# ruc-aimc-lab/GeoFormer

Measured on AMD Instinct MI355X. Metric: image-pairs/sec (640x640), higher is better.
Workload: dtype f16

## Files before the change

geoformer_amd/csrc/k10_conv3x3.hip:

```cpp
#include <type_traits>

#include "gf_common.h"

namespace {

constexpr int TW = 32, PW = TW + 2;
constexpr int C10_FRAG = 1024;
constexpr int P_OFF = 0;
enum { C10_NONE = 0, C10_RELU = 1, C10_LEAKY = 2 };

struct ConvArgs {
    const void* x;
    const void* wstream;
    const float* shift;
    const void* res;
    void* out;
    const void* zeros;
    int N, H, W, act;
    float slope;
    int tiles_x, tiles_y, ntiles;
    int Hi, Wi;
};

template <int NT, int NW, bool REM = false, bool S2 = false>
struct ConvGeo {
    static constexpr int PB = NT <= 4 ? 2 : 1;
    static constexpr int TH = NW * PB, PH = S2 ? TH + 1 : TH + 2;
    static constexpr int PIECES = (PH * PW + 15) / 16;
    static constexpr int PLANE_BYTES = PIECES * 1024;
    static constexpr int PATCH_BYTES = S2 ? 4 * PLANE_BYTES : PIECES * 1024;
    static constexpr int W10_OFF = S2 ? PATCH_BYTES : 2 * PATCH_BYTES;
    static_assert(!S2 || PB == 1, "the stride-2 form is built for the wide outputs (one row per wave)");
#ifndef K10_BS
#define K10_BS 6
#endif
    static constexpr int BLOCK_STEPS = S2 ? 3 : (NW == 8 && PB == 1) ? K10_BS : 6;
    static constexpr int FR = BLOCK_STEPS * NT;
    static constexpr int WBLK = FR * C10_FRAG;
    static constexpr int SHIFT_OFF = W10_OFF + 2 * WBLK;
    static constexpr int RPIECES = (PH * PW + 63) / 64;
    static constexpr int R_OFF = SHIFT_OFF + NT * 32 * 4 + 16;
    static constexpr int LDS = R_OFF + (REM ? RPIECES * 1024 : 0);
    static_assert(LDS <= 160 * 1024, "LDS budget");
};

struct ConvRsrc {
    __amdgpu_buffer_rsrc_t r;
};
__device__ __forceinline__ ConvRsrc conv_rsrc(const void* p, unsigned bytes) {
    return ConvRsrc{__builtin_amdgcn_make_buffer_rsrc(const_cast<void*>(p), 0, (int)bytes, 0x00020000)};
}
__device__ __forceinline__ void conv_lds_dma(const ConvRsrc& rs, char* dst, int voffset, int soffset) {
    __builtin_amdgcn_raw_ptr_buffer_load_lds(rs.r, (__attribute__((address_space(3))) void*)dst, 16, voffset, soffset, 0, 0);
}
template <int NT, int NW, bool S2 = false>
__device__ __forceinline__ void conv_dma_block(const ConvRsrc& ws, char* smem, int b, int slot, int wave, int lane, int i0 = 0, int i1 = 1 << 20) {
    using G = ConvGeo<NT, NW, false, S2>;
    asm volatile("" : "+v"(lane));
    char* dst = smem + G::W10_OFF + slot * G::WBLK;
#pragma unroll
    for (int i = 0; i < (G::FR + NW - 1) / NW; ++i) {
        const int f = wave + NW * i;
        if (i >= i0 && i < i1 && (NW * (i + 1) <= G::FR || f < G::FR)) conv_lds_dma(ws, dst + f * C10_FRAG, lane * 16, b * G::WBLK + f * C10_FRAG);
    }
}

template <typename T, int CIN, int NT, int NW>
__device__ __forceinline__ void conv_dma_patch(const ConvArgs& a, const ConvRsrc& xs, char* smem, int buf, int n, int y0, int x0, int c, int wave,
                                               int lane, int i0 = 0, int i1 = 1 << 20) {
    using G = ConvGeo<NT, NW>;
    asm volatile("" : "+v"(lane));
    char* dst = smem + P_OFF + buf * G::PATCH_BYTES;
    const int sbase = ((n * a.Hi + y0 - 1) * a.Wi + x0 - 1) * CIN + 32 * c;
#pragma unroll
    for (int i = 0; i < (G::PIECES + NW - 1) / NW; ++i) {
        const int piece = wave + NW * i;
        if (i >= i0 && i < i1 && (NW * (i + 1) <= G::PIECES || piece < G::PIECES)) {
            const int q = piece * 16 + (lane >> 2), slot = (lane & 3) ^ ((q >> 1) & 3);
            const int pr = q / PW, pc = q - pr * PW;
            const bool in = (unsigned)(y0 - 1 + pr) < (unsigned)a.Hi && (unsigned)(x0 - 1 + pc) < (unsigned)a.Wi && q < G::PH * PW;
            int off = (sbase + (pr * a.Wi + pc) * CIN + 8 * slot) * (int)sizeof(T);
            asm volatile("" : "+v"(off));
            conv_lds_dma(xs, dst + piece * 1024, in ? off : 0x7FFFFFF0, 0);
        }
    }
}

template <typename T, int CIN, int NT, int NW>
__device__ __forceinline__ void conv_dma_plane(const ConvArgs& a, const ConvRsrc& xs, char* smem, int plane, int n, int y0, int x0, int c, int wave,
                                               int lane) {
    using G = ConvGeo<NT, NW, false, true>;
    asm volatile("" : "+v"(lane));
    char* dst = smem + P_OFF + plane * G::PLANE_BYTES;
    const int py = plane >> 1, px = plane & 1;
    const int iy0 = 2 * y0 - 1 + py, ix0 = 2 * x0 - 1 + px;
    const int sbase = ((n * a.Hi + iy0) * a.Wi + ix0) * CIN + 32 * c;
#pragma unroll
    for (int i = 0; i < (G::PIECES + NW - 1) / NW; ++i) {
        const int piece = wave + NW * i;
        if (piece < G::PIECES) {
            const int q = piece * 16 + (lane >> 2), slot = (lane & 3) ^ ((q >> 1) & 3);
            const int pr = q / PW, pc = q - pr * PW;
            const bool in = (unsigned)(iy0 + 2 * pr) < (unsigned)a.Hi && (unsigned)(ix0 + 2 * pc) < (unsigned)a.Wi && q < G::PH * PW;
            int off = (sbase + 2 * (pr * a.Wi + pc) * CIN + 8 * slot) * (int)sizeof(T);
            asm volatile("" : "+v"(off));
            conv_lds_dma(xs, dst + piece * 1024, in ? off : 0x7FFFFFF0, 0);
        }
    }
}

template <typename T, int CIN, int NT, int NW>
__device__ __forceinline__ void conv_dma_patch_rem(const ConvArgs& a, const ConvRsrc& xs, char* smem, int n, int y0, int x0, int wave, int lane) {
    using G = ConvGeo<NT, NW, true>;
    asm volatile("" : "+v"(lane));
    char* dst = smem + G::R_OFF;
    const int sbase = ((n * a.Hi + y0 - 1) * a.Wi + x0 - 1) * CIN + 192;
#pragma unroll
    for (int i = 0; i < (G::RPIECES + NW - 1) / NW; ++i) {
        const int piece = wave + NW * i;
        if (piece < G::RPIECES) {
            const int q = piece * 64 + lane;
            const int pr = q / PW, pc = q - pr * PW;
            const bool in = (unsigned)(y0 - 1 + pr) < (unsigned)a.Hi && (unsigned)(x0 - 1 + pc) < (unsigned)a.Wi && q < G::PH * PW;
            const int off = sbase + (pr * a.Wi + pc) * CIN;
            conv_lds_dma(xs, dst + piece * 1024, in ? off * (int)sizeof(T) : 0x7FFFFFF0, 0);
        }
    }
}

#ifndef K10_TRACE
#define K10_TRACE 0
#endif
#ifdef K10_EXP_NOSTORE
#define K10_STORE_OK (a.slope == 12345.f)
#else
#define K10_STORE_OK true
#endif
#if K10_TRACE
__device__ long long k10_trace[256 * 8 * 8 * 16];
#define K10_T(slot) do { if (lane == 0 && it < 8) k10_trace[((blockIdx.x * 8 + it) * 8 + wave) * 16 + (slot)] = (long long)__builtin_amdgcn_s_memtime(); } while (0)
__device__ long long k10_trace2[256 * 8 * 32];
#define K10_T2(slot) do { if (lane == 0 && it == 4 && c == 1) k10_trace2[(blockIdx.x * 8 + wave) * 32 + (slot)] = (long long)__builtin_amdgcn_s_memtime(); } while (0)
#else
#define K10_T(slot)
#define K10_T2(slot)
#endif

template <typename T, int CIN, int COUT, int NW, bool PADL, bool REM = false, bool S2 = false>
__global__ __launch_bounds__(NW * 64) void conv3x3_kernel(ConvArgs a) {
    using Mm = Mma16<T>;
    using Frag = typename Mm::Frag;
    using G = ConvGeo<COUT / 32, NW, REM, S2>;
    static_assert(!(S2 && REM), "no remainder form at stride 2");
    using V4 = gf_vec<T, 4>;
    using V8 = gf_vec<T, 8>;
    static_assert(!REM || CIN == 224, "the remainder form is built for 224-channel inputs");
    constexpr int NT = COUT / 32, NCH = REM ? 6 : CIN / 32, BS = G::BLOCK_STEPS, BPC = 18 / BS, RBPC = 6 / BS;
    constexpr int NBLK = NCH * BPC + (REM ? RBPC : 0);
    constexpr int PB = G::PB, TH = G::TH;
    constexpr int NSTORE = PB * 2 * NT;
    constexpr int WP = (G::FR + NW - 1) / NW, PP = (G::PIECES + NW - 1) / NW, PPMIN = G::PIECES / NW;
#ifndef K10_DEAL
#define K10_DEAL 0
#endif
    constexpr bool DEAL = K10_DEAL != 0;
    constexpr int WS = !DEAL ? 1 : WP <= 3 ? WP : 4, PS0 = DEAL ? WS : 0, PS = DEAL ? BS - WS : 1;
    auto wbeg = [](int k) { return k >= WS ? WP : k * (WP / WS) + (k < WP % WS ? k : WP % WS); };
    auto pbeg = [](int k) { return k >= PS ? PP : k * (PP / PS) + (k < PP % PS ? k : PP % PS); };
    extern __shared__ __attribute__((aligned(16))) char smem[];
    const int tid = threadIdx.x, lane = tid & 63, wave = __builtin_amdgcn_readfirstlane(tid >> 6);
    const int lp = lane & 15, g4 = lane >> 4;
    const ConvRsrc ws = conv_rsrc(a.wstream, (unsigned)NBLK * G::WBLK);
    const ConvRsrc xs = conv_rsrc(a.x, (unsigned)a.N * a.Hi * a.Wi * CIN * (unsigned)sizeof(T));
    const ConvRsrc rres = conv_rsrc(a.res, (unsigned)a.N * a.H * a.W * COUT * (unsigned)sizeof(T));
    const ConvRsrc rout = conv_rsrc(a.out, (unsigned)a.N * a.H * a.W * COUT * (unsigned)sizeof(T));
    typedef unsigned v4u __attribute__((ext_vector_type(4)));
    float* shiftv = reinterpret_cast<float*>(smem + G::SHIFT_OFF);
    for (int i = tid; i < COUT; i += NW * 64) shiftv[i] = a.shift ? a.shift[i] : 0.f;
    if (tid == 0) shiftv[COUT] = a.act == C10_LEAKY ? a.slope : 1.f;
    if (NW == 8 && wave >= 4) __builtin_amdgcn_s_setprio(1);

    auto decode = [&](int t, int& n, int& y0, int& x0) {
        const int per = a.tiles_x * a.tiles_y;
        n = t / per;
        const int r = t - n * per, ty = r / a.tiles_x;
        y0 = ty * TH;
        x0 = (r - ty * a.tiles_x) * TW;
    };
    const int n_none = a.N;
    const int xq0 = PB * wave * PW + lp;
    int swz = 0;
#pragma unroll
    for (int d = 0; d < 8; ++d) swz |= (g4 ^ (((xq0 + d) >> 1) & 3)) << (2 * d);
    const int xbase = xq0 * 64;
    Frag wa[NT], wb[NT], xa[2 * PB], xb[2 * PB];
    auto load_w = [&](Frag (&f)[NT], int slot, int s, bool second_half) {
        const char* p = smem + G::W10_OFF + slot * G::WBLK + s * NT * C10_FRAG + lane * 16;
#pragma unroll
        for (int t = 0; t < NT; ++t)
            if (!(PADL && second_half && t == NT - 1)) f[t] = *reinterpret_cast<const Frag*>(p + t * C10_FRAG);
    };
    auto load_x = [&](Frag (&f)[2 * PB], int buf, int tap) {
        constexpr int s2_plane[9] = {0, 0, 0, 0, 1, 1, 2, 2, 3}, s2_dy[9] = {0, 0, 1, 1, 0, 1, 0, 0, 0}, s2_dx[9] = {0, 1, 0, 1, 0, 0, 0, 1, 0};
        const int ky = S2 ? s2_dy[tap] : tap / 3, kx = S2 ? s2_dx[tap] : tap - 3 * (tap / 3);
        const char* p = smem + P_OFF + (S2 ? s2_plane[tap] * G::PLANE_BYTES : buf * G::PATCH_BYTES);
#ifndef K10_SWZ_TABLE
#define K10_SWZ_TABLE 1
#endif
        if constexpr (K10_SWZ_TABLE != 0) {
            int tb = swz, xb = xbase;
            asm volatile("" : "+v"(tb), "+v"(xb));
#pragma unroll
            for (int bb = 0; bb < 2 * PB; ++bb) {
                const int c = ((bb >> 1) + ky) * PW + 16 * (bb & 1) + kx;
                const int slot = __builtin_amdgcn_ubfe(tb, 2 * (c & 7), 2);
                f[bb] = *reinterpret_cast<const Frag*>(p + (xb + (slot << 4)) + c * 64);
            }
        } else {
        int xq = xq0;
        asm volatile("" : "+v"(xq));
#pragma unroll
        for (int bb = 0; bb < 2 * PB; ++bb) {
            const int q = xq + ((bb >> 1) + ky) * PW + 16 * (bb & 1) + kx;
            f[bb] = *reinterpret_cast<const Frag*>(p + q * 64 + ((g4 ^ ((q >> 1) & 3)) << 4));
        }
        }
    };

    auto load_xr = [&](Frag (&f)[2 * PB], int ks) {
        const char* p = smem + G::R_OFF;
        int xq = xq0;
        asm volatile("" : "+v"(xq));
// ... 19 lines not shown
        decode(tile0, n, y0, x0);
        if constexpr (S2) {
#pragma unroll
            for (int pl = 0; pl < 4; ++pl) conv_dma_plane<T, CIN, NT, NW>(a, xs, smem, pl, n, y0, x0, 0, wave, lane);
        } else {
            conv_dma_patch<T, CIN, NT, NW>(a, xs, smem, 0, n, y0, x0, 0, wave, lane);
        }
        conv_dma_block<NT, NW, S2>(ws, smem, 0, 0, wave, lane);
        conv_dma_block<NT, NW, S2>(ws, smem, 1, 1, wave, lane);
        asm volatile("s_waitcnt vmcnt(0) lgkmcnt(0)" ::: "memory");
        __syncthreads();
    }
    int it = -1;
    for (int tile = tile0; tile < xend; tile += xper) {
        int n, y0, x0;
        decode(tile, n, y0, x0);
        const int nxt_tile = tile + xper;
        const bool has_next = nxt_tile < xend;
        int n2 = n_none, y2 = 0, x2 = 0;
        if (has_next) decode(nxt_tile, n2, y2, x2);
        ++it;
        K10_T(0);
        load_w(wa, wslot, 0, false);
        load_x(xa, pbuf, 0);
        v4f acc[2 * PB][2 * NT];
        int il = lane;
        asm volatile("" : "+v"(il));
#pragma unroll
        for (int ct = 0; ct < 2 * NT; ++ct) {
            const float4 sh = *reinterpret_cast<const float4*>(shiftv + 32 * (ct >> 1) + 4 * (ct & 1) + 8 * (il >> 4));
#pragma unroll
            for (int bb = 0; bb < 2 * PB; ++bb) acc[bb][ct] = v4f{sh.x, sh.y, sh.z, sh.w};
        }
        auto chunk = [&](auto rem_c, int c) {
            constexpr bool R = decltype(rem_c)::value;
            constexpr int NTS = R ? 6 : 18;
            const int blk0 = R ? NCH * BPC : c * BPC;
            const bool tile_ends = R || (!REM && c + 1 == NCH);
            const bool rem_next = !R && REM && c + 1 == NCH;
#pragma unroll
            for (int ts = 0; ts < NTS; ++ts) {
                const int tap = ts >> 1, hf = ts & 1;
                Frag (&cw)[NT] = (ts & 1) ? wb : wa;
                Frag (&nw)[NT] = (ts & 1) ? wa : wb;
                Frag (&cx)[2 * PB] = (tap & 1) ? xb : xa;
                Frag (&nx)[2 * PB] = (tap & 1) ? xa : xb;
                const int kslot = (ts + 1) % BS;
                if constexpr (!R) K10_T2(ts);
                auto dma_slot = [&]() {
                    if (kslot < WS && !(ts == NTS - 1 && tile_ends)) {
                        if (ts >= BS - 1 || R || c > 0) {
                            const int nb = blk0 + (ts + 1) / BS + 1;
                            conv_dma_block<NT, NW, S2>(ws, smem, nb < NBLK ? nb : has_next ? nb - NBLK : NBLK, wslot ^ 1, wave, lane, wbeg(kslot), wbeg(kslot + 1));
                        }
                    }
                    if constexpr (S2) {
                        if (kslot == 0 && ts >= 8) {
                            const bool same = c + 1 < NCH;
                            conv_dma_plane<T, CIN, NT, NW>(a, xs, smem, (ts - 8) / 3, same ? n : n2, same ? y0 : y2, same ? x0 : x2, same ? c + 1 : 0, wave, lane);
                        }
                    } else if (!R && ts >= BS - 1 + PS0 && ts < BS - 1 + PS0 + PS) {
                        const int kp = ts - (BS - 1 + PS0);
                        const bool same = c + 1 < NCH;
                        conv_dma_patch<T, CIN, NT, NW>(a, xs, smem, pbuf ^ 1, same ? n : n2, same ? y0 : y2, same ? x0 : x2, same ? c + 1 : 0,
                                                       wave, lane, pbeg(kp), pbeg(kp + 1));
                        if constexpr (REM) {
                            if (c == 0 && kp == PS - 1) conv_dma_patch_rem<T, CIN, NT, NW>(a, xs, smem, n, y0, x0, wave, lane);
                        }
                    }
                };
                if (kslot == 0) {
                    const bool first_turn = !R && ts == BS - 1 && c == 0;
                    if (first_turn) K10_T(12);
                    if (first_turn && it > 0) asm volatile("s_waitcnt vmcnt(%0)" ::"n"(NSTORE) : "memory");
                    else if (!S2 && !R && ts == 2 * BS - 1) asm volatile("s_waitcnt vmcnt(%0)" ::"n"(PPMIN) : "memory");
                    else if (S2 && (ts >= 11 || (ts == BS - 1 && c > 0))) asm volatile("s_waitcnt vmcnt(%0)" ::"n"(PPMIN) : "memory");
                    else asm volatile("s_waitcnt vmcnt(0)" ::: "memory");
                    if (first_turn) K10_T(13);
                    if constexpr (!R) K10_T2(20 + ts / BS);
                    __builtin_amdgcn_s_barrier();
#ifdef K10_STAGGER
                    if (NW == 8 && wave >= 4) __builtin_amdgcn_s_sleep(K10_STAGGER);
#endif
                    if constexpr (!R) K10_T2(24 + ts / BS);
                    if (first_turn) K10_T(14);
                    wslot ^= 1;
                    if (ts == NTS - 1 && tile_ends) {
                        const int nb = blk0 + ts / BS + 2;
                        conv_dma_block<NT, NW, S2>(ws, smem, has_next ? nb - NBLK : NBLK, wslot ^ 1, wave, lane);
                    }
                    if (!DEAL) {
                        dma_slot();
                        if (first_turn) K10_T(15);
                    }
                    __builtin_amdgcn_sched_barrier(0);
                }
                if (DEAL && wave < 4) {
                    dma_slot();
                    __builtin_amdgcn_sched_barrier(0);
                }
                if (ts < NTS - 1 || !tile_ends) {
                    load_w(nw, wslot, (ts + 1) % BS, ((ts + 1) & 1) != 0);
                    if (hf) {
                        if constexpr (R) {
                            if (ts < NTS - 1) load_xr(nx, tap + 1);
                        } else {
                            if (ts < NTS - 1) load_x(nx, pbuf, tap + 1);
                            else if (rem_next) load_xr(nx, 0);
                            else load_x(nx, pbuf ^ 1, 0);
                        }
                    }
                }
#pragma unroll
                for (int bb = 0; bb < 2 * PB; ++bb)
#pragma unroll
                    for (int t = 0; t < NT; ++t)
                        if (!(PADL && hf == 1 && t == NT - 1)) Mm::mma(cw[t], cx[bb], acc[bb][hf * NT + t]);
                if (DEAL && wave >= 4) {
                    __builtin_amdgcn_sched_barrier(0);
                    dma_slot();
                }
                __builtin_amdgcn_sched_barrier(0);
            }
            if (!tile_ends) {
#pragma unroll
                for (int bb = 0; bb < 2 * PB; ++bb) xa[bb] = xb[bb];
            }
            if constexpr (!R) pbuf ^= 1;
            if constexpr (!R) K10_T2(18);
        };
#pragma unroll 1
        for (int c = 0; c < NCH; ++c) {
            chunk(std::integral_constant<bool, false>{}, c);
            K10_T(2 + c);
        }
        if constexpr (REM) chunk(std::integral_constant<bool, true>{}, NCH);
        K10_T(10);
        auto epilogue = [&](auto has_res_c, auto mode_c) {
            constexpr bool HAS_RES = decltype(has_res_c)::value;
            constexpr int MODE = decltype(mode_c)::value;
            int el = lane;
            asm volatile("" : "+v"(el));
            const float neg_k = MODE == 3 ? shiftv[COUT + (el >> 6)] : 1.f;
            const int odd = el & 1, ey = y0 + PB * wave;
            const int exa = x0 + (el & 14), exo = x0 + (el & 15);
            const int ebase = ((n * a.H + ey) * a.W + x0) * COUT * (int)sizeof(T) + 16 * (el >> 4);
#ifndef K10_XCHG_WIDE
#define K10_XCHG_WIDE 1
#endif
            constexpr int NB = 2 * PB, NM = (PB == 2 || K10_XCHG_WIDE) ? NT / 2 : 0, NL = NT - 2 * NM;
            constexpr bool LONE = NL != 0;
            int voa[NB], vob[NB], vol[LONE ? NB : 1];
#pragma unroll
            for (int bb = 0; bb < NB; ++bb) {
                const int rowoff = ((bb >> 1) * a.W + 16 * (bb & 1)) * COUT * (int)sizeof(T);
                const bool iny = ey + (bb >> 1) < a.H;
                voa[bb] = iny && exa + 16 * (bb & 1) < a.W ? ebase + rowoff + (el & 14) * COUT * (int)sizeof(T) + 64 * odd : 0x7FFFFFF0;
                vob[bb] = iny && exa + 1 + 16 * (bb & 1) < a.W ? ebase + rowoff + ((el & 14) + 1) * COUT * (int)sizeof(T) + 64 * odd : 0x7FFFFFF0;
                if constexpr (LONE) vol[bb] = iny && exo + 16 * (bb & 1) < a.W ? ebase + rowoff + (el & 15) * COUT * (int)sizeof(T) + 64 * (2 * NM) : 0x7FFFFFF0;
            }
            auto pack8 = [](const v4f& lo, const v4f& hi) {
                return V8{(T)lo[0], (T)lo[1], (T)lo[2], (T)lo[3], (T)hi[0], (T)hi[1], (T)hi[2], (T)hi[3]};
            };
            auto exchange = [&](const V8& p0, const V8& p1, V8& da, V8& db) {
                const v4u u0 = __builtin_bit_cast(v4u, p0), u1 = __builtin_bit_cast(v4u, p1);
                v4u ua, ub;
#pragma unroll
// ... 28 lines not shown
            auto load8 = [&](int vo, int imm) { return __builtin_bit_cast(V8, __builtin_amdgcn_raw_buffer_load_b128(rres.r, vo + imm, 0, 0)); };
            auto store8 = [&](const V8& o, int vo, int imm) {
                if (K10_STORE_OK) __builtin_amdgcn_raw_buffer_store_b128(__builtin_bit_cast(v4u, o), rout.r, vo + imm, 0, 0);
            };
            constexpr int BATCH = (HAS_RES && MODE == 3) ? 1 : NB;
#pragma unroll
            for (int b0 = 0; b0 < NB; b0 += BATCH) {
                V8 ra[HAS_RES ? BATCH : 1][HAS_RES ? NM : 1], rb[HAS_RES ? BATCH : 1][HAS_RES ? NM : 1], rlone[HAS_RES && LONE ? BATCH : 1][LONE ? NL : 1];
                if constexpr (HAS_RES) {
#pragma unroll
                    for (int bq = 0; bq < BATCH; ++bq) {
#pragma unroll
                        for (int m = 0; m < NM; ++m) {
                            ra[bq][m] = load8(voa[b0 + bq], 128 * m);
                            rb[bq][m] = load8(vob[b0 + bq], 128 * m);
                        }
                        if constexpr (LONE) {
#pragma unroll
                            for (int q = 0; q < NL; ++q) rlone[bq][q] = load8(vol[b0 + bq], 64 * q);
                        }
                    }
                }
#pragma unroll
                for (int bq = 0; bq < BATCH; ++bq) {
                    const int bb = b0 + bq;
#pragma unroll
                    for (int m = 0; m < NM; ++m) {
                        V8 da, db;
                        exchange(pack8(acc[bb][4 * m], acc[bb][4 * m + 1]), pack8(acc[bb][4 * m + 2], acc[bb][4 * m + 3]), da, db);
                        store8(finish(da, ra[HAS_RES ? bq : 0][HAS_RES ? m : 0]), voa[bb], 128 * m);
                        store8(finish(db, rb[HAS_RES ? bq : 0][HAS_RES ? m : 0]), vob[bb], 128 * m);
                        if constexpr (MODE >= 2) __builtin_amdgcn_sched_barrier(0);
                    }
                    if constexpr (LONE) {
#pragma unroll
                        for (int q = 0; q < NL; ++q) {
                            store8(finish(pack8(acc[bb][4 * NM + 2 * q], acc[bb][4 * NM + 2 * q + 1]), rlone[HAS_RES ? bq : 0][q]), vol[bb], 64 * q);
                            if constexpr (MODE >= 2) __builtin_amdgcn_sched_barrier(0);
                        }
                    }
                }
            }
        };
        using std::integral_constant;
        auto by_res = [&](auto mode_c) {
            if (a.res) epilogue(integral_constant<bool, true>{}, mode_c);
            else epilogue(integral_constant<bool, false>{}, mode_c);
        };
        if constexpr (std::is_same<T, _Float16>::value) {
            if (a.act == C10_RELU) by_res(integral_constant<int, 0>{});
            else if (a.act == C10_NONE) by_res(integral_constant<int, 1>{});
            else by_res(integral_constant<int, 3>{});
        } else {
            if (a.act == C10_RELU) by_res(integral_constant<int, 2>{});
            else by_res(integral_constant<int, 3>{});
        }
        K10_T(11);
    }
    asm volatile("s_waitcnt vmcnt(0) lgkmcnt(0)" ::: "memory");
}

#if K10_TRACE
}
extern "C" int gf_debug_k10_trace(long long* out) {
    return hipMemcpyFromSymbol(out, HIP_SYMBOL(k10_trace), sizeof(k10_trace)) == hipSuccess ? 0 : -1;
}
extern "C" int gf_debug_k10_trace2(long long* out) {
    return hipMemcpyFromSymbol(out, HIP_SYMBOL(k10_trace2), sizeof(k10_trace2)) == hipSuccess ? 0 : -1;
}
namespace {
#endif

template <typename T, int CIN, int COUT, int NW, bool PADL, bool REM = false, bool S2 = false>
int conv_launch(ConvArgs a, hipStream_t st) {
    using G = ConvGeo<COUT / 32, NW, REM, S2>;
    static std::atomic<uint64_t> attr{0};
    if (gf_first_use_on_device(attr))
        (void)hipFuncSetAttribute((const void*)conv3x3_kernel<T, CIN, COUT, NW, PADL, REM, S2>, hipFuncAttributeMaxDynamicSharedMemorySize, G::LDS);
    a.tiles_x = (a.W + TW - 1) / TW;
    a.tiles_y = (a.H + G::TH - 1) / G::TH;
    const long nt = (long)a.N * a.tiles_x * a.tiles_y;
    if (nt >= (1l << 31)) return -2;
    a.ntiles = (int)nt;
    conv3x3_kernel<T, CIN, COUT, NW, PADL, REM, S2><<<a.ntiles < 256 ? a.ntiles : 256, NW * 64, G::LDS, st>>>(a);
    return 0;
}

template <typename T, int CIN, int COUT, bool PADL = false, bool REM = false, bool S2 = false>
int conv_launch_w(const ConvArgs& a, hipStream_t st) {
    return conv_launch<T, CIN, COUT, 8, PADL, REM, S2>(a, st);
}

template <typename T>
int conv_dispatch(const ConvArgs& a, int cin, int cout, bool padl, bool rem, bool s2, hipStream_t st) {
    if (s2) {
        if (cin == 128 && cout == 224 && padl) return conv_launch_w<T, 128, 224, true, false, true>(a, st);
        if (cin == 128 && cout == 224) return conv_launch_w<T, 128, 224, false, false, true>(a, st);
        if (cin == 224 && cout == 256) return conv_launch_w<T, 224, 256, false, false, true>(a, st);
        return -1;
    }
    if (rem) {
        if (cin == 224 && cout == 224 && padl) return conv_launch_w<T, 224, 224, true, true>(a, st);
        if (cin == 224 && cout == 128 && !padl) return conv_launch_w<T, 224, 128, false, true>(a, st);
        return -1;
    }
    if (cin == 128 && cout == 128) return conv_launch_w<T, 128, 128>(a, st);
    if (cin == 224 && cout == 224 && padl) return conv_launch_w<T, 224, 224, true>(a, st);
    if (cin == 256 && cout == 224 && padl) return conv_launch_w<T, 256, 224, true>(a, st);
    if (cin == 224 && cout == 224) return conv_launch_w<T, 224, 224>(a, st);
    if (cin == 224 && cout == 128) return conv_launch_w<T, 224, 128>(a, st);
    if (cin == 256 && cout == 256) return conv_launch_w<T, 256, 256>(a, st);
    if (cin == 256 && cout == 224) return conv_launch_w<T, 256, 224>(a, st);
    if (cin == 128 && cout == 224) return conv_launch_w<T, 128, 224>(a, st);
    if (cin == 224 && cout == 256) return conv_launch_w<T, 224, 256>(a, st);
    return -1;
}

}

extern "C" int gf_conv3x3s2_supported(int cin, int cout) { return (cin == 128 && cout == 224) || (cin == 224 && cout == 256); }

extern "C" int gf_conv3x3_supported(int cin, int cout) {
    return (cin == 128 && (cout == 128 || cout == 224)) || (cin == 224 && (cout == 224 || cout == 128 || cout == 256)) || (cin == 256 && (cout == 256 || cout == 224));
}

extern "C" int gf_conv3x3_nhwc(const void* x, const void* wstream, const float* shift, const void* residual, void* out,
                               const void* zeros, int N, int H, int W, int cin, int cout, int act, float slope, int dtype,
                               void* stream) {
    GF_CHECK_ARG(x && wstream && out && zeros, "null pointer");
    GF_CHECK_ARG(N > 0 && H > 0 && W > 0, "empty problem");
    GF_CHECK_ARG(dtype == GF_F16 || dtype == GF_BF16, "built for 16-bit maps");
    const bool padl = (act & GF_CONV_PAD16) != 0;
    const bool rem = (act & GF_CONV_REM8) != 0;
    const bool s2 = (act & GF_CONV_S2) != 0;
    act &= ~(GF_CONV_PAD16 | GF_CONV_REM8 | GF_CONV_S2);
    GF_CHECK_ARG(s2 ? gf_conv3x3s2_supported(cin, cout) : gf_conv3x3_supported(cin, cout),
                 "no kernel for these channel counts (see gf_conv3x3_supported / gf_conv3x3s2_supported)");
    GF_CHECK_ARG(!rem || (!s2 && cin == 224 && ((cout == 224 && padl) || (cout == 128 && !padl))),
                 "GF_CONV_REM8 is built for stride 1, Cin = 224 with Cout = 224 | GF_CONV_PAD16 or Cout = 128");
    GF_CHECK_ARG(!padl || cout == 224, "GF_CONV_PAD16 belongs to 224-wide outputs");
    GF_CHECK_ARG(act >= C10_NONE && act <= C10_LEAKY, "unknown activation");
    GF_CHECK_ARG(act != C10_LEAKY || (slope >= 0.f && slope <= 1.f), "LeakyReLU slope must lie in [0, 1]");
    GF_CHECK_ARG((uintptr_t)x % 16 == 0 && (uintptr_t)out % 16 == 0 && (uintptr_t)residual % 16 == 0 && (uintptr_t)wstream % 16 == 0 &&
                     (uintptr_t)zeros % 16 == 0, "tensors must be 16-byte aligned");
    GF_CHECK_ARG((long)N * H * W * (cin > cout ? cin : cout) * 2 < 0x7FFFFFF0l, "maps of 2 GiB or more are not supported (32-bit buffer offsets)");
    const int Ho = s2 ? (H - 1) / 2 + 1 : H, Wo = s2 ? (W - 1) / 2 + 1 : W;
    ConvArgs a{x, wstream, shift, residual, out, zeros, N, Ho, Wo, act, slope, 0, 0, 0, H, W};
    hipStream_t st = (hipStream_t)stream;
    const double cin_w = cin == 224 ? 196.0 : cin, cout_w = cout == 224 ? 196.0 : cout;
    void* pt = gf_prof_begin("conv3x3", st, 2.0 * N * (double)Ho * Wo * cin_w * cout_w * 9.0);
    const int rc = dtype == GF_F16 ? conv_dispatch<_Float16>(a, cin, cout, padl, rem, s2, st) : conv_dispatch<gf_bf16>(a, cin, cout, padl, rem, s2, st);
    gf_prof_end("conv3x3", pt, st);
    GF_CHECK_ARG(rc == 0, "dispatch failed");
    GF_CHECK_LAUNCH();
    return GF_OK;
}
```

geoformer_amd/fused.py:

```python
import ctypes

import torch

from . import _lib
from ._lib import check
from .ops import _DTYPES, _contig, _dt, _need_cuda, _p, _rows2d, _stream, _ws

_IDX = {}


def _frag_index(order, device):
    key = (order, str(device))
    if key not in _IDX:
        lane = torch.arange(64, device=device)[:, None]
        j = torch.arange(8, device=device)[None, :]
        h = lane >> 5
        if order == 'std':
            koff = 8 * h + j
        else:
            koff = 8 * (j >> 2) + 4 * h + (j & 3)
        _IDX[key] = (koff, (lane & 31).expand(64, 8))
    return _IDX[key]


# ... 128 lines not shown
        raise ValueError('gf_fine_layer: x and src must be [Nw, Lw, 128] tensors of one 16-bit dtype')
    x = _contig(x)
    src = x if src is x else _contig(src)
    if out is None:
        out = torch.empty_like(x)
    elif out.shape != x.shape or out.dtype != x.dtype or not out.is_contiguous():
        raise ValueError('out must be a contiguous tensor of the result shape and dtype')
    if Nw == 0:
        return out
    check(_lib.lib().gf_fine_layer(_p(x), _p(src), _p(out), _dt(x), Nw, Lw, _p(wstream), _p(ln_params), float(eps1), float(eps2),
                                   float(attn_eps), _stream()), 'gf_fine_layer')
    return out


_ZEROS = {}


def pack_conv3x3_stream(w, rem8=False, s2=False):
    cout, cin = w.shape[:2]
    nt = cout // 32
    dev = w.device
    lane = torch.arange(64, device=dev)
    row, kg = lane % 16, lane // 16
    ct = torch.arange(2, device=dev)[:, None, None] * nt + torch.arange(nt, device=dev)[None, :, None]
    co = 32 * (ct // 2) + 4 * (ct % 2) + (8 * (row // 4) + row % 4)[None, None, :]
    kk = 8 * kg[:, None] + torch.arange(8, device=dev)[None, :]
    full = 192 if rem8 else cin
    if rem8 and (cin != 224 or bool(w[:, 200:].any())):
        raise ValueError('rem8 packs a 224-channel convolution whose input channels 200.. have zero weights')
    wt = w[:, :full].reshape(cout, full // 32, 32, 9)
    if s2:
        if rem8:
            raise ValueError('no remainder form at stride 2')
        wt = wt[..., torch.tensor([0, 2, 6, 8, 1, 7, 3, 5, 4], device=dev)]
    g = wt[co[:, :, :, None], :, kk[None, None, :, :], :]
    out = g.permute(4, 5, 0, 1, 2, 3).contiguous().reshape(-1)
    if not rem8:
        return out
    wr = torch.zeros(cout, 8, 12, dtype=w.dtype, device=dev)
    wr[:, :, :9] = w[:, 192:200].reshape(cout, 8, 9)
    j = torch.arange(8, device=dev)
    tap = 4 * torch.arange(3, device=dev)[:, None] + kg[None, :]
    r = wr[co[None, :, :, :, None], j[None, None, None, None, :], tap[:, None, None, :, None]]
    return torch.cat([out, r.contiguous().reshape(-1)])


def pack_lateral_frags(w):
    w = w.reshape(w.shape[0], w.shape[1])
    cout, cin = w.shape
    dev = w.device
    lane = torch.arange(64, device=dev)
    row, kg = lane % 16, lane // 16
    ct = torch.arange(cout // 16, device=dev)[:, None]
    co = 32 * (ct // 2) + 4 * (ct % 2) + (8 * (row // 4) + row % 4)[None, :]
    kk = 8 * kg[:, None] + torch.arange(8, device=dev)[None, :]
    kc = torch.arange(cin // 32, device=dev)
    return w[co[None, :, :, None], (32 * kc[:, None, None, None] + kk[None, None, :, :])].contiguous().reshape(-1)


def lateral_supported(cin, cout):
    return bool(_lib.lib().gf_lateral_supported(int(cin), int(cout)))


def lateral_upsample_add(x, wfrag, cout, lo):
    _need_cuda(x, wfrag, lo)
    if x.dim() != 4 or not x.is_contiguous(memory_format=torch.channels_last) or not lo.is_contiguous(memory_format=torch.channels_last):
        raise ValueError('lateral_upsample_add expects channels_last [N, C, H, W] tensors')
    N, cin, H, W = x.shape
    if lo.shape[:2] != (N, cout) or lo.dtype != x.dtype or wfrag.dtype != x.dtype:
        raise ValueError('lo must be [N, cout, h, w] of the dtype of x and of the fragments')
    out = torch.empty(N, cout, H, W, dtype=x.dtype, device=x.device, memory_format=torch.channels_last)
    check(_lib.lib().gf_lateral_upsample_add_nhwc(_p(x), _p(wfrag), _p(lo), _p(out), N, lo.shape[2], lo.shape[3], H, W, cin, cout,
                                                  _dt(x), _stream()), 'gf_lateral_upsample_add_nhwc')
    return out


def conv3x3_supported(cin, cout):
    return bool(_lib.lib().gf_conv3x3_supported(int(cin), int(cout)))


CONV_PAD16 = 0x100
CONV_REM8 = 0x200
CONV_S2 = 0x400


def conv3x3s2_supported(cin, cout):
    return bool(_lib.lib().gf_conv3x3s2_supported(int(cin), int(cout)))


def conv3x3(x, wstream, cout, shift=None, residual=None, act=0, slope=0.01, pad16=False, rem8=False, stride=1):
    _need_cuda(x, wstream)
    if x.dim() != 4 or not x.is_contiguous(memory_format=torch.channels_last):
        raise ValueError('conv3x3 expects a channels_last [N, C, H, W] tensor')
    N, cin, H, W = x.shape
    if stride not in (1, 2):
        raise ValueError('stride 1 or 2')
    Ho, Wo = ((H - 1) // 2 + 1, (W - 1) // 2 + 1) if stride == 2 else (H, W)
    out = torch.empty(N, cout, Ho, Wo, dtype=x.dtype, device=x.device, memory_format=torch.channels_last)
    if residual is not None and (residual.shape != out.shape or residual.dtype != x.dtype or
                                 not residual.is_contiguous(memory_format=torch.channels_last)):
        raise ValueError('residual must be a channels_last tensor of the output shape and dtype')
    z = _ZEROS.get(x.device)
    if z is None:
        z = _ZEROS[x.device] = torch.zeros(256, dtype=torch.uint8, device=x.device)
    check(_lib.lib().gf_conv3x3_nhwc(_p(x), _p(wstream), _p(shift), _p(residual), _p(out), _p(z), N, H, W, cin, cout,
                                     int(act) | (CONV_PAD16 if pad16 else 0) | (CONV_REM8 if rem8 else 0) | (CONV_S2 if stride == 2 else 0),
                                     float(slope), _dt(x), _stream()), 'gf_conv3x3_nhwc')
    return out


def conv3x3_wgrad(x, dy, cin=None, cout=None):
    _need_cuda(x, dy)
    for t in (x, dy):
        if t.dim() != 4 or not t.is_contiguous(memory_format=torch.channels_last):
            raise ValueError('conv3x3_wgrad expects channels_last [N, C, H, W] tensors')
    N, cx, H, W = x.shape
    cy = dy.shape[1]
    if dy.shape[0] != N or tuple(dy.shape[2:]) != (H, W) or dy.dtype != x.dtype:
        raise ValueError('x and dy must agree in batch, size and dtype')
    cin, cout = int(cin or cx), int(cout or cy)
    dw = torch.empty(cout, cin, 3, 3, dtype=torch.float32, device=x.device)
    L_ = _lib.lib()
    ws = _ws.get('k10wgrad', L_.gf_conv3x3_wgrad_workspace_bytes(N, H, W, cin, cout), x.device)
    check(L_.gf_conv3x3_wgrad_nhwc(_p(x), _p(dy), _dt(x), N, H, W, cx, cy, cin, cout, _p(dw), _p(ws), ws.numel(), _stream()), 'gf_conv3x3_wgrad_nhwc')
    return dw
```

include/geoformer_hip.h:

```cpp
#ifndef GEOFORMER_HIP_H_
#define GEOFORMER_HIP_H_

#include <stddef.h>
#include <stdint.h>

#ifdef __cplusplus
extern "C" {
#endif

typedef enum { GF_OK = 0, GF_ERR_INVALID_ARGUMENT = -1, GF_ERR_WORKSPACE = -2, GF_ERR_LAUNCH = -3 } gf_status;
typedef enum { GF_F32 = 0, GF_F16 = 1, GF_BF16 = 2 } gf_dtype;

#define GF_ABI_VERSION 4
int gf_abi_version(void);
const char* gf_last_error(void);

void gf_profile_enable(int on);
void gf_profile_filter(const char* tag);
int gf_profile_collect(const char* tag, double* total_ms, int* count, double* work);

size_t gf_dual_softmax_workspace_bytes(int N, int L, int S);
int gf_dual_softmax_match_only_supported(int dtype, int L, int S, int C, int masked, int force_one);
int gf_dual_softmax_conf_at(const void* f0, const void* f1, int dtype, int N, int L, int S, int C, float temperature,
                            const int64_t* b, const int64_t* i, const int64_t* j, int P, float* out, void* workspace,
                            size_t workspace_bytes, void* stream);
int gf_dual_softmax_match(const void* f0, const void* f1, int dtype, int N, int L, int S, int C,
                          const uint8_t* mask0, const uint8_t* mask1, float temperature, float thr,
                          int force_one, int w0c, int w1c, float scale, const float* scale0,
                          const float* scale1, float* conf, int64_t* b_ids, int64_t* i_ids,
                          int64_t* j_ids, float* mconf, float* mkpts0_c, float* mkpts1_c,
                          int32_t* counts, void* workspace, size_t workspace_bytes, void* stream);

size_t gf_linear_wgrad_workspace_bytes(long T, int cout, int cin);
int gf_linear_wgrad(const void* dy, long lddy, const void* x, long ldx, int dtype, long T, int cout, int cin, float* dw,
                    long lddw, int accumulate, void* workspace, size_t workspace_bytes, void* stream);
int gf_layernorm_forward(const void* y, int dtype, long T, int C, const float* gamma, const float* beta, float eps, void* out,
                         float* stats, void* stream);
size_t gf_layernorm_backward_workspace_bytes(int C);
int gf_layernorm_backward(const void* dout, const void* y, const float* stats, int dtype, long T, int C, const float* gamma, void* dy,
                          float* dgamma, float* dbeta, int accumulate, void* workspace, size_t workspace_bytes, void* stream);
int gf_activation_backward(const void* dh, const void* h, void* dz, size_t n, int kind, int dtype, void* stream);

int gf_fine_match_backward(const void* f0, const void* f1, int dtype, int M, int WW, int C, float temperature, const float* dconf,
                           void* df0, void* df1, void* stream);
size_t gf_linear_attention_backward_workspace_bytes(int N, int L, int S, int H);
int gf_linear_attention_backward(const void* q, const void* k, const void* v, const void* dout, int dtype, int N, int L, int S, int H,
                                 int D, long ldq, long ldk, long ldv, long ldo, const uint8_t* q_mask, const uint8_t* kv_mask, float eps,
                                 void* dq, void* dk, void* dv, void* workspace, size_t workspace_bytes, void* stream);
int gf_window_linear_attention_backward(const void* q, const void* k, const void* v, const void* dout, int dtype, int Nw, int Lw,
                                        float eps, void* dq, void* dk, void* dv, void* stream);

size_t gf_conv3x3_wgrad_workspace_bytes(int N, int H, int W, int cin, int cout);
int gf_conv3x3_wgrad_nhwc(const void* x, const void* dy, int dtype, int N, int H, int W, int cx, int cy, int cin, int cout, float* dw,
                          void* workspace, size_t workspace_bytes, void* stream);

int gf_full_attention_train_forward(const void* q, const void* k, const void* v, int dtype, int N, int L, int S, int H, int D, long ldq,
                                    long ldk, long ldv, float softmax_temp, void* out, long ldo, float* lse, void* stream);
size_t gf_full_attention_backward_workspace_bytes(int N, int L, int H);
int gf_full_attention_backward(const void* q, const void* k, const void* v, const void* out, const void* dout, const float* lse,
                               int dtype, int N, int L, int S, int H, int D, long ldq, long ldk, long ldv, long ldo, long lddo,
                               float softmax_temp, void* dq, void* dk, void* dv, void* workspace, size_t workspace_bytes,
                               void* stream);

size_t gf_coarse_loss_workspace_bytes(int N, int L, int S);
int gf_coarse_loss_forward(const void* f0, const void* f1, int dtype, int N, int L, int S, int C, const uint8_t* mask0,
                           const uint8_t* mask1, float temperature, const int64_t* pos_b, const int64_t* pos_i, const int64_t* pos_j, int P,
                           const float* pos_weight, float alpha, float gamma, float* pos_conf, float* pos_loss,
                           float* pos_grad, void* workspace, size_t workspace_bytes, void* stream);
int gf_coarse_loss_backward(int N, int L, int S, int C, const uint8_t* mask0, const uint8_t* mask1, float temperature,
                            const int64_t* pos_b, const int64_t* pos_i,
                            const int64_t* pos_j, int P, const float* pos_grad, float scale, const float* scale_dev,
                            float* d_f0, float* d_f1, void* workspace, size_t workspace_bytes, void* stream);

int gf_pos_encode(const void* x, int x_dtype, long sn, long sc, long sh, long sw, const float* pe,
                  void* out, int out_dtype, int N, int C, int H, int W, void* stream);

size_t gf_linear_attention_workspace_bytes(int N, int S, int H, int D);
int gf_linear_attention(const void* q, const void* k, const void* v, int dtype, int N, int L, int S, int H,
                        int D, long ldq, long ldk, long ldv, const uint8_t* q_mask, const uint8_t* kv_mask,
                        float eps, void* out, void* workspace, size_t workspace_bytes, void* stream);

size_t gf_encoder_kv_workspace_bytes(int N, int S);
int gf_encoder_kv_state(const void* src, long ld, int dtype, int N, int S, const uint8_t* kv_mask,
                        const void* wstream_kv, float* kv_state, void* workspace, size_t workspace_bytes,
                        void* stream);
int gf_encoder_layer(const void* x, long ldx, const void* msg, long ldm, const float* kv_state, int S,
                     const uint8_t* q_mask, float attn_eps, const void* wstream, const float* ln_params, float eps1,
                     float eps2, int activation, const int32_t* row_flag, int flag_rows, void* out, long ldo, int dtype,
                     int N, int L, void* stream);
int gf_encoder_layer_kv(const void* x, long ldx, const float* kv_state, int S, const uint8_t* q_mask, float attn_eps,
                        const void* wstream, const float* ln_params, float eps1, float eps2, int activation, void* out,
                        long ldo, int dtype, int N, int L, const void* wstream_tail, int tail_first, float* kv_state_out,
                        void* workspace, size_t workspace_bytes, void* stream);

int gf_fine_layer(const void* x, const void* src, void* out, int dtype, int Nw, int Lw, const void* wstream,
                  const float* ln_params, float eps1, float eps2, float attn_eps, void* stream);

#define GF_CONV_PAD16 0x100
#define GF_CONV_REM8 0x200
#define GF_CONV_S2 0x400
int gf_conv3x3_supported(int cin, int cout);
int gf_conv3x3s2_supported(int cin, int cout);
int gf_conv3x3_nhwc(const void* x, const void* wstream, const float* shift, const void* residual, void* out,
                    const void* zeros, int N, int H, int W, int cin, int cout, int act, float slope, int dtype,
                    void* stream);

int gf_linear(const void* a1, long lda1, int k1, const void* a2, long lda2, int k2, const void* w,
              const float* bias, const void* rowgroup_bias, int rowgroup_rows, int epilogue,
              const float* ln_gamma, const float* ln_beta, float ln_eps, const void* residual, long ldres,
              const int32_t* row_flag, int flag_rows, void* out, long ldo, int dtype, int M, int N,
              void* stream);

size_t gf_ransac_workspace_bytes(int N, int iters);
int gf_ransac_homography(const float* mkpts0_c, const float* mkpts1_c, const int32_t* counts, int N,
                         int capacity, float scale, const float* scale0, const float* scale1, float thr,
                         int iters, uint32_t seed, int min_points, int integer_keypoints, float* kp0, float* kp1, double* M,
                         float* M_f32, float* Minv_f32, int32_t* valid, uint8_t* keep, void* workspace,
                         size_t workspace_bytes, void* stream);
int gf_ransac_homography_v2(const float* mkpts0_c, const float* mkpts1_c, const int32_t* counts, int N,
                            int capacity, float scale, const float* scale0, const float* scale1, float thr,
                            int iters, uint32_t seed, int min_points, int integer_keypoints, float* kp0, float* kp1, double* M,
                            float* M_f32, float* Minv_f32, int32_t* valid, uint8_t* keep, void* workspace,
                            size_t workspace_bytes, void* stream, int lm_iters);

int gf_window_geometry(const float* H, const int32_t* valid, int N, int hq, int wq, int Himg, int Wimg,
                       int wk, int scale, int window_size, const float* window_scale, int32_t* win,
                       int32_t* kps_or_null, float* warped_or_null, void* stream);

int gf_inlier_index(const float* kp0, const float* kp1, const uint8_t* keep, const int32_t* counts, int N,
                    int L, int S, int w0, int w1, int scale, uint8_t* map0, uint8_t* map1, int32_t* idx0,
                    int32_t* idx1, int32_t* nidx, void* stream);

size_t gf_self_attention_workspace_bytes(int N, int L, int dtype);
int gf_self_attention_gathered(const void* q, const void* kmap, const void* vmap, int dtype, int N, int L, int H,
                               int D, long ldq, long ldk, long ldv, const int32_t* idx, long idx_stride,
                               const int32_t* nkeys, int nkeys_stride, void* out, void* workspace,
                               size_t workspace_bytes, void* stream);

int gf_window_cross_attention(const void* q, const void* kmap, const void* vmap, int dtype, int N, int L, int S,
                              int H, int D, long ldq, long ldk, long ldv, const int32_t* win, int WW,
                              const int32_t* valid, void* out, void* stream);
int gf_window_cross_attention_backward(const void* q, const void* kmap, const void* vmap, const void* dout, int dtype, int N, int L,
                                       int S, int H, int D, long ldq, long ldk, long ldv, const int32_t* win, int WW, void* dq,
                                       float* dk, float* dv, void* stream);
size_t gf_window_cross_attention_backward_workspace_bytes(int N, int L, int WW);
int gf_window_cross_attention_backward_gather(const void* q, const void* kmap, const void* vmap, const void* dout, int dtype, int N, int L,
                                              int S, int H, int D, long ldq, long ldk, long ldv, const int32_t* win, int WW,
                                              const int32_t* entries, const int32_t* offsets, void* dq, void* dk, void* dv, void* workspace,
                                              size_t workspace_bytes, void* stream);
int gf_window_cross_attention_tiled(const void* q, const void* kmap, const void* vmap, int dtype, int N, int hq, int wq,
                                    int hk, int wk, int H, int D, long ldq, long ldk, long ldv, const int32_t* win,
                                    int WW, const int32_t* valid, void* out, void* stream);

int gf_fine_gather(const void* feat_f0, const void* feat_f1, int feat_dtype, const long* strides0,
                   const long* strides1, int H0, int W0, int H1, int W1, int C, const void* feat_c0,
                   const void* feat_c1, int dtype, int L, int S, int CC, const int64_t* b_ids,
                   const int64_t* i_ids, const int64_t* j_ids, int M, int w0c, int w1c, int stride, int window,
                   void* win_out, void* ccat_out, void* stream);

int gf_bias_act_nhwc(const void* x, const float* bias, const void* residual, void* out, long pixels, int C, int act,
                     float slope, int dtype, void* stream);
int gf_upsample_add_nhwc(const void* lo, const void* hi, void* out, int N, int h, int w, int H, int W, int C,
                         int dtype, void* stream);
int gf_upsample_bilinear_backward_nhwc(const void* dhi, void* dlo, int N, int h, int w, int H, int W, int C, int dtype, void* stream);
int gf_conv1x1_upsample_add_nhwc(const void* x, const void* w, const void* lo, void* out, int N, int h, int wl, int H,
                                 int W, int Cin, int Cout, int dtype, void* stream);

int gf_lateral_supported(int cin, int cout);
int gf_lateral_upsample_add_nhwc(const void* x, const void* wfrag, const void* lo, void* out, int N, int h, int w, int H, int W,
                                 int cin, int cout, int dtype, void* stream);
int gf_conv1x1_nhwc(const void* x, const void* w, void* out, int N, int H, int W, int Cin, int Cout, int stride, int dtype,
                    void* stream);
int gf_stem_conv7x7(const void* image, int image_dtype, const float* weight, const float* shift, void* out, int N,
                    int H, int W, int C, void* stream);
int gf_stem_conv7x7_dt(const void* image, int image_dtype, const float* weight, const float* shift, void* out, int out_dtype, int N,
                       int H, int W, int C, void* stream);

size_t gf_fine_match_workspace_bytes(int M);
int gf_fine_match(const void* f0, const void* f1, int dtype, int M, int WW, int C, float temperature, float thr,
                  const int64_t* b_ids, const float* mkpts0_c, const float* mkpts1_c, float coarse_scale,
                  float c2f_scale, float fine_scale, const float* scale0, const float* scale1,
                  float* fine_matrix, float* mkpts0_f, float* mkpts1_f, float* mconf, int64_t* m_bids,
                  int32_t* count, void* workspace, size_t workspace_bytes, void* stream);
// ... 6 lines not shown
```

Baseline: 730.4.

## Add four-wave conv3x3 variant running two workgroups per CU for small grids

Adds a 4-wave form of the 3x3 conv kernel whose LDS footprint is capped at 80 KiB with 3-step weight blocks, so two workgroups can share a CU. The dispatcher picks it for selected channel pairs when the tile count is small (at most 256, or between 512 and 768) and an occupancy query confirms two blocks fit. The aim is better CU fill and latency hiding where the 8-wave grid leaves CUs underused or unevenly loaded. The cost is smaller weight blocks, which means more barrier and DMA turns. A new one_domain flag lets callers force the 8-wave path.

```diff
diff --git a/geoformer_amd/csrc/k10_conv3x3.hip b/geoformer_amd/csrc/k10_conv3x3.hip
--- a/geoformer_amd/csrc/k10_conv3x3.hip
+++ b/geoformer_amd/csrc/k10_conv3x3.hip
@@ -34,14 +34,15 @@
 #ifndef K10_BS
 #define K10_BS 6
 #endif
-    static constexpr int BLOCK_STEPS = S2 ? 3 : (NW == 8 && PB == 1) ? K10_BS : 6;
+    static constexpr int BLOCK_STEPS = (S2 || NW == 4) ? 3 : PB == 1 ? K10_BS : 6;
     static constexpr int FR = BLOCK_STEPS * NT;
     static constexpr int WBLK = FR * C10_FRAG;
     static constexpr int SHIFT_OFF = W10_OFF + 2 * WBLK;
     static constexpr int RPIECES = (PH * PW + 63) / 64;
     static constexpr int R_OFF = SHIFT_OFF + NT * 32 * 4 + 16;
     static constexpr int LDS = R_OFF + (REM ? RPIECES * 1024 : 0);
-    static_assert(LDS <= 160 * 1024, "LDS budget");
+    static_assert(LDS <= (NW == 4 ? 80 : 160) * 1024, "LDS budget (two four-wave workgroups share the CU's 160 KiB)");
+    static_assert(!(S2 && NW == 4), "the stride-2 planes (80 KB) leave no room for a second workgroup");
 };
 
 struct ConvRsrc {
@@ -137,9 +138,9 @@
 #define K10_STORE_OK true
 #endif
 #if K10_TRACE
-__device__ long long k10_trace[256 * 8 * 8 * 16];
+__device__ long long k10_trace[512 * 8 * 8 * 16];
 #define K10_T(slot) do { if (lane == 0 && it < 8) k10_trace[((blockIdx.x * 8 + it) * 8 + wave) * 16 + (slot)] = (long long)__builtin_amdgcn_s_memtime(); } while (0)
-__device__ long long k10_trace2[256 * 8 * 32];
+__device__ long long k10_trace2[512 * 8 * 32];
 #define K10_T2(slot) do { if (lane == 0 && it == 4 && c == 1) k10_trace2[(blockIdx.x * 8 + wave) * 32 + (slot)] = (long long)__builtin_amdgcn_s_memtime(); } while (0)
 #else
 #define K10_T(slot)
@@ -147,7 +148,7 @@
 #endif
 
 template <typename T, int CIN, int COUT, int NW, bool PADL, bool REM = false, bool S2 = false>
-__global__ __launch_bounds__(NW * 64) void conv3x3_kernel(ConvArgs a) {
+__global__ __launch_bounds__(NW * 64, NW == 4 ? 2 : 1) void conv3x3_kernel(ConvArgs a) {
     using Mm = Mma16<T>;
     using Frag = typename Mm::Frag;
     using G = ConvGeo<COUT / 32, NW, REM, S2>;
@@ -333,7 +334,7 @@
 #ifdef K10_STAGGER
                     if (NW == 8 && wave >= 4) __builtin_amdgcn_s_sleep(K10_STAGGER);
 #endif
-                    if constexpr (!R) K10_T2(24 + ts / BS);
+                    if constexpr (!R) K10_T2(26 + ts / BS);
                     if (first_turn) K10_T(14);
                     wslot ^= 1;
                     if (ts == NTS - 1 && tile_ends) {
@@ -528,37 +529,71 @@
     const long nt = (long)a.N * a.tiles_x * a.tiles_y;
     if (nt >= (1l << 31)) return -2;
     a.ntiles = (int)nt;
-    conv3x3_kernel<T, CIN, COUT, NW, PADL, REM, S2><<<a.ntiles < 256 ? a.ntiles : 256, NW * 64, G::LDS, st>>>(a);
+    constexpr int MAXWG = NW == 4 ? 512 : 256;
+    conv3x3_kernel<T, CIN, COUT, NW, PADL, REM, S2><<<a.ntiles < MAXWG ? a.ntiles : MAXWG, NW * 64, G::LDS, st>>>(a);
     return 0;
 }
 
+template <typename T, int CIN, int COUT, bool PADL, bool REM>
+bool conv_two_fit() {
+    static std::atomic<uint64_t> known{0}, fits{0};
+    int dev = 0;
+    if (hipGetDevice(&dev) != hipSuccess || dev < 0 || dev > 63) return false;
+    const uint64_t bit = 1ull << dev;
+    if (!(known.load(std::memory_order_acquire) & bit)) {
+        using G = ConvGeo<COUT / 32, 4, REM>;
+        const void* k = (const void*)conv3x3_kernel<T, CIN, COUT, 4, PADL, REM, false>;
+        int nb = 0;
+        if (hipFuncSetAttribute(k, hipFuncAttributeMaxDynamicSharedMemorySize, G::LDS) == hipSuccess &&
+            hipOccupancyMaxActiveBlocksPerMultiprocessor(&nb, k, 4 * 64, G::LDS) == hipSuccess && nb >= 2)
+            fits.fetch_or(bit, std::memory_order_release);
+        (void)hipGetLastError();
+        known.fetch_or(bit, std::memory_order_release);
+    }
+    return (fits.load(std::memory_order_acquire) & bit) != 0;
+}
+
+#ifndef K10_TWO_ALL
+#define K10_TWO_ALL 0
+#endif
+constexpr bool conv_has_two(int cin, int cout, bool padl, bool rem) {
+    return K10_TWO_ALL || (cin == 128 && cout == 128) || (cin == 224 && cout == 224 && padl && rem) || (cin == 224 && cout == 128 && rem) ||
+           (cin == 256 && cout == 256) || (cin == 256 && cout == 224 && padl);
+}
+
 template <typename T, int CIN, int COUT, bool PADL = false, bool REM = false, bool S2 = false>
-int conv_launch_w(const ConvArgs& a, hipStream_t st) {
+int conv_launch_w(const ConvArgs& a, bool one_domain, hipStream_t st) {
+    if constexpr (!S2 && conv_has_two(CIN, COUT, PADL, REM)) {
+        constexpr int TH4 = ConvGeo<COUT / 32, 4, REM>::TH;
+        const long t4 = (long)a.N * ((a.W + TW - 1) / TW) * ((a.H + TH4 - 1) / TH4);
+        if (!one_domain && (K10_TWO_ALL || t4 <= 256 || (t4 > 512 && t4 <= 768)) && conv_two_fit<T, CIN, COUT, PADL, REM>())
+            return conv_launch<T, CIN, COUT, 4, PADL, REM, false>(a, st);
+    }
     return conv_launch<T, CIN, COUT, 8, PADL, REM, S2>(a, st);
 }
 
 template <typename T>
-int conv_dispatch(const ConvArgs& a, int cin, int cout, bool padl, bool rem, bool s2, hipStream_t st) {
+int conv_dispatch(const ConvArgs& a, int cin, int cout, bool padl, bool rem, bool s2, bool one_domain, hipStream_t st) {
     if (s2) {
-        if (cin == 128 && cout == 224 && padl) return conv_launch_w<T, 128, 224, true, false, true>(a, st);
-        if (cin == 128 && cout == 224) return conv_launch_w<T, 128, 224, false, false, true>(a, st);
-        if (cin == 224 && cout == 256) return conv_launch_w<T, 224, 256, false, false, true>(a, st);
+        if (cin == 128 && cout == 224 && padl) return conv_launch_w<T, 128, 224, true, false, true>(a, one_domain, st);
+        if (cin == 128 && cout == 224) return conv_launch_w<T, 128, 224, false, false, true>(a, one_domain, st);
+        if (cin == 224 && cout == 256) return conv_launch_w<T, 224, 256, false, false, true>(a, one_domain, st);
         return -1;
     }
     if (rem) {
-        if (cin == 224 && cout == 224 && padl) return conv_launch_w<T, 224, 224, true, true>(a, st);
-        if (cin == 224 && cout == 128 && !padl) return conv_launch_w<T, 224, 128, false, true>(a, st);
+        if (cin == 224 && cout == 224 && padl) return conv_launch_w<T, 224, 224, true, true>(a, one_domain, st);
+        if (cin == 224 && cout == 128 && !padl) return conv_launch_w<T, 224, 128, false, true>(a, one_domain, st);
         return -1;
     }
-    if (cin == 128 && cout == 128) return conv_launch_w<T, 128, 128>(a, st);
-    if (cin == 224 && cout == 224 && padl) return conv_launch_w<T, 224, 224, true>(a, st);
-    if (cin == 256 && cout == 224 && padl) return conv_launch_w<T, 256, 224, true>(a, st);
-    if (cin == 224 && cout == 224) return conv_launch_w<T, 224, 224>(a, st);
-    if (cin == 224 && cout == 128) return conv_launch_w<T, 224, 128>(a, st);
-    if (cin == 256 && cout == 256) return conv_launch_w<T, 256, 256>(a, st);
-    if (cin == 256 && cout == 224) return conv_launch_w<T, 256, 224>(a, st);
-    if (cin == 128 && cout == 224) return conv_launch_w<T, 128, 224>(a, st);
-    if (cin == 224 && cout == 256) return conv_launch_w<T, 224, 256>(a, st);
+    if (cin == 128 && cout == 128) return conv_launch_w<T, 128, 128>(a, one_domain, st);
+    if (cin == 224 && cout == 224 && padl) return conv_launch_w<T, 224, 224, true>(a, one_domain, st);
+    if (cin == 256 && cout == 224 && padl) return conv_launch_w<T, 256, 224, true>(a, one_domain, st);
+    if (cin == 224 && cout == 224) return conv_launch_w<T, 224, 224>(a, one_domain, st);
+    if (cin == 224 && cout == 128) return conv_launch_w<T, 224, 128>(a, one_domain, st);
+    if (cin == 256 && cout == 256) return conv_launch_w<T, 256, 256>(a, one_domain, st);
+    if (cin == 256 && cout == 224) return conv_launch_w<T, 256, 224>(a, one_domain, st);
+    if (cin == 128 && cout == 224) return conv_launch_w<T, 128, 224>(a, one_domain, st);
+    if (cin == 224 && cout == 256) return conv_launch_w<T, 224, 256>(a, one_domain, st);
     return -1;
 }
 
@@ -579,7 +614,8 @@
     const bool padl = (act & GF_CONV_PAD16) != 0;
     const bool rem = (act & GF_CONV_REM8) != 0;
     const bool s2 = (act & GF_CONV_S2) != 0;
-    act &= ~(GF_CONV_PAD16 | GF_CONV_REM8 | GF_CONV_S2);
+    const bool one_domain = (act & GF_CONV_ONE_DOMAIN) != 0;
+    act &= ~(GF_CONV_PAD16 | GF_CONV_REM8 | GF_CONV_S2 | GF_CONV_ONE_DOMAIN);
     GF_CHECK_ARG(s2 ? gf_conv3x3s2_supported(cin, cout) : gf_conv3x3_supported(cin, cout),
                  "no kernel for these channel counts (see gf_conv3x3_supported / gf_conv3x3s2_supported)");
     GF_CHECK_ARG(!rem || (!s2 && cin == 224 && ((cout == 224 && padl) || (cout == 128 && !padl))),
@@ -595,7 +631,7 @@
     hipStream_t st = (hipStream_t)stream;
     const double cin_w = cin == 224 ? 196.0 : cin, cout_w = cout == 224 ? 196.0 : cout;
     void* pt = gf_prof_begin("conv3x3", st, 2.0 * N * (double)Ho * Wo * cin_w * cout_w * 9.0);
-    const int rc = dtype == GF_F16 ? conv_dispatch<_Float16>(a, cin, cout, padl, rem, s2, st) : conv_dispatch<gf_bf16>(a, cin, cout, padl, rem, s2, st);
+    const int rc = dtype == GF_F16 ? conv_dispatch<_Float16>(a, cin, cout, padl, rem, s2, one_domain, st) : conv_dispatch<gf_bf16>(a, cin, cout, padl, rem, s2, one_domain, st);
     gf_prof_end("conv3x3", pt, st);
     GF_CHECK_ARG(rc == 0, "dispatch failed");
     GF_CHECK_LAUNCH();
diff --git a/geoformer_amd/fused.py b/geoformer_amd/fused.py
--- a/geoformer_amd/fused.py
+++ b/geoformer_amd/fused.py
@@ -234,13 +234,14 @@
 CONV_PAD16 = 0x100
 CONV_REM8 = 0x200
 CONV_S2 = 0x400
+CONV_ONE_DOMAIN = 0x800
 
 
 def conv3x3s2_supported(cin, cout):
     return bool(_lib.lib().gf_conv3x3s2_supported(int(cin), int(cout)))
 
 
-def conv3x3(x, wstream, cout, shift=None, residual=None, act=0, slope=0.01, pad16=False, rem8=False, stride=1):
+def conv3x3(x, wstream, cout, shift=None, residual=None, act=0, slope=0.01, pad16=False, rem8=False, stride=1, one_domain=False):
     _need_cuda(x, wstream)
     if x.dim() != 4 or not x.is_contiguous(memory_format=torch.channels_last):
         raise ValueError('conv3x3 expects a channels_last [N, C, H, W] tensor')
@@ -256,8 +257,8 @@
     if z is None:
         z = _ZEROS[x.device] = torch.zeros(256, dtype=torch.uint8, device=x.device)
     check(_lib.lib().gf_conv3x3_nhwc(_p(x), _p(wstream), _p(shift), _p(residual), _p(out), _p(z), N, H, W, cin, cout,
-                                     int(act) | (CONV_PAD16 if pad16 else 0) | (CONV_REM8 if rem8 else 0) | (CONV_S2 if stride == 2 else 0),
-                                     float(slope), _dt(x), _stream()), 'gf_conv3x3_nhwc')
+                                     int(act) | (CONV_PAD16 if pad16 else 0) | (CONV_REM8 if rem8 else 0) | (CONV_S2 if stride == 2 else 0) |
+                                     (CONV_ONE_DOMAIN if one_domain else 0), float(slope), _dt(x), _stream()), 'gf_conv3x3_nhwc')
     return out
 
 
diff --git a/include/geoformer_hip.h b/include/geoformer_hip.h
--- a/include/geoformer_hip.h
+++ b/include/geoformer_hip.h
@@ -99,6 +99,7 @@
 #define GF_CONV_PAD16 0x100
 #define GF_CONV_REM8 0x200
 #define GF_CONV_S2 0x400
+#define GF_CONV_ONE_DOMAIN 0x800
 int gf_conv3x3_supported(int cin, int cout);
 int gf_conv3x3s2_supported(int cin, int cout);
 int gf_conv3x3_nhwc(const void* x, const void* wstream, const float* shift, const void* residual, void* out,
```

Measured after the change: 731.9 (median of 6 runs). About the same (+0.2%).
